# Hippogriff/prifit

Hardware: AMD Instinct MI355X
Metric: shapes/sec (fwd+bwd) B=24x2048 pts, PointNet++-MSG+ellipsoid fit (higher is better)
Workload: dtype f32; 1 GPU; configs[2]: PointNet++-MSG + mean-shift(10 it, <=25 clusters) + ellipsoid fit + convex loss, B=24x2048 per GPU, fwd+bwd+Adam; global_batch=24, points=2048, parallelism=dp1, cloud=blobs, embedding=clustered, backbone_grad_param=sa1.conv_blocks.0.0.weight, launch=eager

## Files before the change

prifit_amd/build.py:

```python
import os
import subprocess
import sys
from concurrent.futures import ThreadPoolExecutor

HERE = os.path.dirname(os.path.abspath(__file__))
ROOT = os.path.dirname(HERE)
CSRC = os.path.join(HERE, "csrc")
LIBDIR = os.path.join(HERE, "lib")
LIB = os.path.join(LIBDIR, "libprifit_hip.so")
OBJDIR = os.path.join(HERE, "build")
ARCH = "gfx950"

SOURCES = {
    "pointops.hip": ["-ffp-contract=off"],
    "sa_group.hip": ["-ffp-contract=off"],
    "gemm.hip": [],
    "gemm_stream.hip": [],
    "gemm_stream_bwd.hip": [],
    "pool_alg.hip": [],
    "sa_gather_bwd.hip": [],
    "bn.hip": [],
    "meanshift.hip": [],
    "meanshift_fused.hip": [],
    "meanshift_rows.hip": [],
    "meanshift_split.hip": [],
    "fit.hip": [],
    "fit_glue.hip": [],
    "chamfer.hip": ["-ffp-contract=off"],
    "atlas.hip": [],
    "optim.hip": [],
    "augment.hip": ["-ffp-contract=off"],
    "perturb.hip": ["-ffp-contract=off"],
    "seg_metrics.hip": [],
    "infer.hip": [],
    "infer_bf16.hip": [],
    "probe_head.hip": [],
    "edge_conv.hip": [],
    "dgcnn.hip": ["-ffp-contract=off"],
    "comm.hip": [],
}
COMMON = ["-O3", "-std=c++17", "-fPIC", "--offload-arch=" + ARCH, "-I" + os.path.join(ROOT, "include"),
          "-I" + CSRC, "-Wall", "-Wno-unused-function"] + os.environ.get("PRIFIT_BUILD_DEFS", "").split()


def _hipcc():
    for c in (os.environ.get("HIPCC"), "/opt/rocm/bin/hipcc", "hipcc"):
        if c and (os.path.isabs(c) and os.path.exists(c) or not os.path.isabs(c)):
            return c
    raise RuntimeError("hipcc not found")


def _stale(target, deps):
    if not os.path.exists(target):
        return True
    t = os.path.getmtime(target)
    return any(os.path.getmtime(d) > t for d in deps)


def build_library(force=False, verbose=False):
    import fcntl
    os.makedirs(LIBDIR, exist_ok=True)
    os.makedirs(OBJDIR, exist_ok=True)
    with open(os.path.join(LIBDIR, ".build.lock"), "w") as lock:
        fcntl.flock(lock, fcntl.LOCK_EX)
        try:
            return _build_locked(force, verbose)
        finally:
            fcntl.flock(lock, fcntl.LOCK_UN)


def _build_locked(force, verbose):
    headers = [os.path.join(CSRC, f) for f in os.listdir(CSRC) if f.endswith(".h")]
    headers.append(os.path.join(ROOT, "include", "prifit_hip.h"))
    hipcc = _hipcc()
    jobs = []
    objs = []
    for src, extra in SOURCES.items():
        s = os.path.join(CSRC, src)
        o = os.path.join(OBJDIR, src.replace(".hip", ".o"))
        objs.append(o)
        if force or _stale(o, [s] + headers):
            jobs.append([hipcc] + COMMON + extra + ["-c", s, "-o", o])

    def run(cmd):
        if verbose:
            print(" ".join(cmd), flush=True)
        r = subprocess.run(cmd, capture_output=True, text=True)
        if r.returncode != 0:
            raise RuntimeError("hipcc failed:\n%s\n%s" % (" ".join(cmd), r.stderr))
        if verbose and r.stderr.strip():
            print(r.stderr)

    if jobs:
        with ThreadPoolExecutor(max_workers=min(4, len(jobs))) as ex:
            list(ex.map(run, jobs))
    if jobs or force or _stale(LIB, objs):
        tmp = LIB + ".tmp.%d" % os.getpid()
        run([hipcc, "-shared", "-fPIC", "--offload-arch=" + ARCH, "-o", tmp] + objs + ["-ldl"])
        os.replace(tmp, LIB)
    return LIB


if __name__ == "__main__":
    print(build_library(force="--force" in sys.argv, verbose=True))
```

prifit_amd/csrc/gemm.hip:

```cpp
#include <stdlib.h>

#include <type_traits>

#include "common.h"

typedef float f32x16 __attribute__((ext_vector_type(16)));

enum { LAY_NT = 0, LAY_NN = 1, LAY_TN = 2 };
enum { EPI_NONE = 0, EPI_CHORD = 1, EPI_MSKERNEL = 2, EPI_MSBWD = 3, EPI_BNRED = 4 };

struct GemmArgs {
    const float *A, *B;
    float *C;
    int M, N, K;
    long long lda, ldb, ldc;
    long long sA, sB, sC;
    int batch, splitk;
    const float *a_scale, *a_shift;
    const float *b_scale, *b_shift;
    const float *bias;
    long long bias_stride;
    float *stats;
    int epi;
    const float *epi_batch_scalar;
    const float *aux;
    const float *row_add;
    float *a_rowsum;
    long long ldaux, sAux;
    const float *red_scale, *red_shift, *red_mean, *red_invstd;
    long long dA2, dB2;
    int kswitch;
    int accumulate;
    int vecA, vecB;
    int ntiles;
    float *cand;
};

#ifndef GEMM_W8
#define GEMM_W8 6
#endif
constexpr int BK = 32;
constexpr int PAD = 4;

__device__ __forceinline__ float4 ld4(const float *p) { return *reinterpret_cast<const float4 *>(p); }

template <int ROWS, bool KC, bool VEC, bool AFF, int NTH>
struct TileLoader {
    static constexpr int NV = ROWS * BK / 4 / NTH;
    static_assert(NV * NTH * 4 == ROWS * BK, "tile must divide evenly over the threads");
    float4 v[NV];
    const float *ptr[NV];
    int klo[NV];
    int c0[NV];
    unsigned okmask[NV];
    long long step;
    int K, R, cclamp;

    __device__ __forceinline__ void init(const float *__restrict__ base, long long ld, int r0, int R_, int K_)
    {
        K = K_; R = R_;
        step = KC ? (long long)BK : (long long)BK * ld;
#pragma unroll
        for (int p = 0; p < NV; ++p) {
            const int id = threadIdx.x + NTH * p;
            if (KC) {
                const int gr = r0 + id / (BK / 4);
                klo[p] = (id % (BK / 4)) * 4;
                okmask[p] = gr < R ? 0xFu : 0u;
                ptr[p] = base + (long long)(gr < R ? gr : 0) * ld + (klo[p] < K ? klo[p] : 0);
                c0[p] = 0;
            } else {
                klo[p] = id / (ROWS / 4);
                const int gr = r0 + (id % (ROWS / 4)) * 4;
                unsigned m = 0;
#pragma unroll
                for (int j = 0; j < 4; ++j) m |= (gr + j < R) ? (1u << j) : 0u;
                okmask[p] = m;
                c0[p] = m ? gr : 0;
                ptr[p] = base + (long long)klo[p] * ld + c0[p];
            }
        }
    }

    int kload;
    __device__ __forceinline__ void load(int k0, const float *__restrict__, const float *__restrict__)
    {
        kload = k0;
        const int kt = k0 / BK;
#pragma unroll
        for (int p = 0; p < NV; ++p) {
            const int gk = k0 + klo[p];
            const bool kin = gk < K;
            const float *src = ptr[p] + (kin ? (long long)kt * step : 0);
            if (!KC && !kin && klo[p] >= K) src = ptr[p] - (long long)klo[p] * (step / BK);
            if (VEC) {
                v[p] = ld4(src);
            } else {
                float e[4];
#pragma unroll
                for (int j = 0; j < 4; ++j) {
                    const bool ok = KC ? (okmask[p] && (gk + j) < K) : (kin && ((okmask[p] >> j) & 1u));
                    e[j] = src[ok ? j : 0];
                }
                v[p] = make_float4(e[0], e[1], e[2], e[3]);
            }
        }
    }

    __device__ __forceinline__ void finish(const float *__restrict__ scale, const float *__restrict__ shift)
    {
#pragma unroll
        for (int p = 0; p < NV; ++p) {
            const int gk = kload + klo[p];
            const bool kin = gk < K;
            float4 x = v[p];
            if (VEC) {
                if (AFF) {
                    const int cc = KC ? (kin ? gk : 0) : c0[p];
                    const float4 s = ld4(scale + cc), t = ld4(shift + cc);
                    x.x = fmaxf(fmaf(x.x, s.x, t.x), 0.f); x.y = fmaxf(fmaf(x.y, s.y, t.y), 0.f);
                    x.z = fmaxf(fmaf(x.z, s.z, t.z), 0.f); x.w = fmaxf(fmaf(x.w, s.w, t.w), 0.f);
                }
                if (!(kin && okmask[p])) x = make_float4(0.f, 0.f, 0.f, 0.f);
            } else {
                float e[4] = {x.x, x.y, x.z, x.w};
#pragma unroll
                for (int j = 0; j < 4; ++j) {
                    const bool ok = KC ? (okmask[p] && (gk + j) < K) : (kin && ((okmask[p] >> j) & 1u));
                    float val = ok ? e[j] : 0.f;
                    if (AFF && ok) {
                        const int cc = KC ? gk + j : c0[p] + j;
                        val = fmaxf(fmaf(val, scale[cc], shift[cc]), 0.f);
                    }
                    e[j] = val;
                }
                x = make_float4(e[0], e[1], e[2], e[3]);
            }
            v[p] = x;
        }
    }

    __device__ __forceinline__ void shift(long long delta)
    {
#pragma unroll
        for (int p = 0; p < NV; ++p) ptr[p] += delta;
    }

    __device__ __forceinline__ void store(float *__restrict__ lds) const
    {
#pragma unroll
        for (int p = 0; p < NV; ++p) {
            const int id = threadIdx.x + NTH * p;
            if (KC) {
                const int row = id / (BK / 4), kk = (id % (BK / 4)) * 4;
                *reinterpret_cast<float4 *>(lds + row * (BK + PAD) + kk) = v[p];
            } else {
                const int kk = id / (ROWS / 4), row = (id % (ROWS / 4)) * 4;
                *reinterpret_cast<float4 *>(lds + kk * (ROWS + PAD) + row) = v[p];
            }
        }
    }
};

typedef float f32x4v __attribute__((ext_vector_type(4)));
typedef unsigned u32x4v __attribute__((ext_vector_type(4)));
template <int ROWS, bool KC, bool AFF, int NTH>
struct ExactLoader {
    static constexpr int NV = ROWS * BK / 4 / NTH;
    static_assert(NV * NTH * 4 == ROWS * BK, "tile must divide evenly over the threads");
    float4 v[NV];
    int voff[NV];
    int klo[NV], c0[NV];
    const float *base;
    __amdgpu_buffer_rsrc_t rs;
    int step4;
    int kload;

    __device__ __forceinline__ void init(const float *__restrict__ b, long long ld, int r0, int, int)
    {
        base = b;
        rs = __builtin_amdgcn_make_buffer_rsrc(const_cast<float *>(b), 0, 0x7ffffffc, 0x00020000);
        step4 = __builtin_amdgcn_readfirstlane(KC ? BK * 4 : (int)(BK * ld * 4));
#pragma unroll
        for (int p = 0; p < NV; ++p) {
            const int id = threadIdx.x + NTH * p;
            if (KC) {
                klo[p] = (id % (BK / 4)) * 4;
                c0[p] = 0;
                voff[p] = (int)(((long long)(r0 + id / (BK / 4)) * ld + klo[p]) * 4);
            } else {
                klo[p] = id / (ROWS / 4);
                c0[p] = r0 + (id % (ROWS / 4)) * 4;
                voff[p] = (int)(((long long)klo[p] * ld + c0[p]) * 4);
            }
        }
    }
    __device__ __forceinline__ void load(int k0, const float *__restrict__, const float *__restrict__)
    {
        kload = k0;
        const int soff = __builtin_amdgcn_readfirstlane((k0 / BK) * step4);
#pragma unroll
        for (int p = 0; p < NV; ++p) {
            const f32x4v t = __builtin_bit_cast(f32x4v, __builtin_amdgcn_raw_buffer_load_b128(rs, voff[p], soff, 0));
            v[p] = make_float4(t.x, t.y, t.z, t.w);
        }
    }
    __device__ __forceinline__ void finish(const float *__restrict__ scale, const float *__restrict__ shift)
    {
        if (!AFF) return;
#pragma unroll
        for (int p = 0; p < NV; ++p) {
            const int cc = KC ? kload + klo[p] : c0[p];
            const float4 s = ld4(scale + cc), t = ld4(shift + cc);
            float4 x = v[p];
            x.x = fmaxf(fmaf(x.x, s.x, t.x), 0.f); x.y = fmaxf(fmaf(x.y, s.y, t.y), 0.f);
            x.z = fmaxf(fmaf(x.z, s.z, t.z), 0.f); x.w = fmaxf(fmaf(x.w, s.w, t.w), 0.f);
            v[p] = x;
        }
    }
    __device__ __forceinline__ void shift(long long delta)
    {
        base += delta;
        rs = __builtin_amdgcn_make_buffer_rsrc(const_cast<float *>(base), 0, 0x7ffffffc, 0x00020000);
    }
    __device__ __forceinline__ void store(float *__restrict__ lds) const
    {
#pragma unroll
        for (int p = 0; p < NV; ++p) {
            const int id = threadIdx.x + NTH * p;
            if (KC) {
                const int row = id / (BK / 4), kk = (id % (BK / 4)) * 4;
                *reinterpret_cast<float4 *>(lds + row * (BK + PAD) + kk) = v[p];
            } else {
                const int kk = id / (ROWS / 4), row = (id % (ROWS / 4)) * 4;
                *reinterpret_cast<float4 *>(lds + kk * (ROWS + PAD) + row) = v[p];
            }
        }
    }
};

template <int ROWS, bool KC, bool AFF, int NTH>
struct BufLoader {
    static constexpr int NV = ROWS * BK / 4 / NTH;
    static_assert(NV * NTH * 4 == ROWS * BK, "tile must divide evenly over the threads");
    static constexpr int OOBV = 0x7fffffff;
    float4 v[NV];
    int voff[NV];
    int klo[NV], c0[NV];
    __amdgpu_buffer_rsrc_t rs;
    const float *base;
    int step4, K, kload;

    __device__ __forceinline__ void init(const float *__restrict__ b, long long ld, int r0, int R, int K_)
    {
        K = K_;
        base = b;
        rs = __builtin_amdgcn_make_buffer_rsrc(const_cast<float *>(b), 0, 0x7ffffffc, 0x00020000);
        step4 = KC ? BK * 4 : (int)(BK * ld * 4);
#pragma unroll
        for (int p = 0; p < NV; ++p) {
            const int id = threadIdx.x + NTH * p;
            if (KC) {
                const int row = r0 + id / (BK / 4);
                klo[p] = (id % (BK / 4)) * 4;
                c0[p] = 0;
                voff[p] = row < R ? (int)(((long long)row * ld + klo[p]) * 4) : OOBV;
            } else {
                klo[p] = id / (ROWS / 4);
                c0[p] = r0 + (id % (ROWS / 4)) * 4;
                voff[p] = c0[p] < R ? (int)(((long long)klo[p] * ld + c0[p]) * 4) : OOBV;
                if (c0[p] >= R) c0[p] = 0;
            }
        }
    }
    __device__ __forceinline__ void load(int k0, const float *__restrict__, const float *__restrict__) { load(k0); }
    __device__ __forceinline__ void shift(long long delta)
    {
        base += delta;
        rs = __builtin_amdgcn_make_buffer_rsrc(const_cast<float *>(base), 0, 0x7ffffffc, 0x00020000);
    }
    __device__ __forceinline__ void load(int k0)
    {
        kload = k0;
        const int soff = (k0 / BK) * step4;
        if (k0 + BK <= K) {
#pragma unroll
            for (int p = 0; p < NV; ++p) {
                const f32x4v t = __builtin_bit_cast(f32x4v, __builtin_amdgcn_raw_buffer_load_b128(rs, voff[p], soff, 0));
                v[p] = make_float4(t.x, t.y, t.z, t.w);
            }
        } else {
#pragma unroll
            for (int p = 0; p < NV; ++p) {
                const int vo = k0 + klo[p] < K ? voff[p] : OOBV;
                const f32x4v t = __builtin_bit_cast(f32x4v, __builtin_amdgcn_raw_buffer_load_b128(rs, vo, soff, 0));
                v[p] = make_float4(t.x, t.y, t.z, t.w);
            }
        }
    }
    __device__ __forceinline__ void finish(const float *__restrict__ scale, const float *__restrict__ shift)
    {
        if (!AFF) return;
#pragma unroll
        for (int p = 0; p < NV; ++p) {
            const int gk = kload + klo[p];
            const bool ok = voff[p] != OOBV && gk < K;
            const int cc = KC ? (gk < K ? gk : 0) : c0[p];
// ... 420 lines not shown
            const float bias = (g.bias && cok) ? g.bias[col] : 0.f;
            float rs = 0.f, rt = 0.f, rmu = 0.f, ris = 0.f;
            if (RED && cok) { rs = g.red_scale[col]; rt = g.red_shift[col]; rmu = g.red_mean[col]; ris = g.red_invstd[col]; }
            const int c_voff = cok ? (int)(((long long)rbase * g.ldc + col) * 4) : 0x7fffffff;
            const int y_voff = (RED && cok) ? (int)(((long long)rbase * g.ldaux + col) * 4) : 0x7fffffff;
            float kf[16];
            if (RED) {
#pragma unroll
                for (int r = 0; r < 16; ++r) {
                    const int ro = ((r & 3) + 8 * (r >> 2)) * ldy4;
                    kf[r] = __builtin_bit_cast(float, full_rows ? __builtin_amdgcn_raw_buffer_load_b32(yrs, y_voff, ro, 0)
                                                                 : __builtin_amdgcn_raw_buffer_load_b32(yrs, cok ? y_voff + ro : y_voff, 0, 0));
                }
            }
            float vmax = -INFINITY, vmin = INFINITY, v0 = 0.f;
            int imax = 0, imin = 0;
#pragma unroll
            for (int r = 0; r < 16; ++r) {
                const int row = rbase + (r & 3) + 8 * (r >> 2);
                const float v = acc[b][r] + bias;
                const float vs = (cok && (full_rows || row < g.M)) ? v : 0.f;
                if (PMAX) {
                    const int ri = (r & 3) + 8 * (r >> 2) + 4 * lh;
                    const bool rok = full_rows || row < g.M;
                    if (rok && v > vmax) { vmax = v; imax = ri; }
                    if (rok && v < vmin) { vmin = v; imin = ri; }
                }
                if (RED) {
                    const float gm = fmaf(kf[r], rs, rt) > 0.f ? vs : 0.f;
                    csum[b] += gm;
                    csq[b] += gm * ((kf[r] - rmu) * ris);
                } else {
                    csum[b] += vs;
                    if (r == 0) v0 = vs;
                    else if (r == 1) csq[b] = fmaf(v0, v0, vs * vs);
                    else csq[b] = fmaf(vs, vs, csq[b]);
                }
                {
                    const int ro = ((r & 3) + 8 * (r >> 2)) * ldc4;
                    if (full_rows) __builtin_amdgcn_raw_buffer_store_b32(__builtin_bit_cast(unsigned, v), crs, c_voff, ro, 0);
                    else __builtin_amdgcn_raw_buffer_store_b32(__builtin_bit_cast(unsigned, v), crs, cok ? c_voff + ro : c_voff, 0, 0);
                }
            }
            if (PMAX) {
                const float ov = __shfl_xor(vmax, 32, 64), on = __shfl_xor(vmin, 32, 64);
                const int oi = __shfl_xor(imax, 32, 64), oj = __shfl_xor(imin, 32, 64);
                if (ov > vmax || (ov == vmax && oi < imax)) { vmax = ov; imax = oi; }
                if (on < vmin || (on == vmin && oj < imin)) { vmin = on; imin = oj; }
                const int blk_row = m0 + wm0;
                if (lh == 0 && cok && blk_row < g.M) {
                    float *cd = g.cand + (long long)(blk_row >> 5) * 4 * g.N + col;
                    cd[0] = vmax; cd[g.N] = __int_as_float(imax); cd[2 * g.N] = vmin; cd[3 * g.N] = __int_as_float(imin);
                }
            }
        }
        PERS_STAMP(3);
        if (g.stats) {
            float *red = lds;
#pragma unroll
            for (int b = 0; b < TN; ++b) {
                const float s = csum[b] + __shfl_xor(csum[b], 32, 64);
                const float q = csq[b] + __shfl_xor(csq[b], 32, 64);
                if (lh == 0) {
                    red[(wmi * 2 + 0) * BN + wn0 + 32 * b + li] = s;
                    red[(wmi * 2 + 1) * BN + wn0 + 32 * b + li] = q;
                }
            }
            __syncthreads();
            for (int t = threadIdx.x; t < 2 * BN; t += NTH) {
                const int which = t / BN, c = t - which * BN;
                float s = 0.f;
#pragma unroll
                for (int w = 0; w < BM / WM; ++w) s += red[(w * 2 + which) * BN + c];
                if (n0 + c < g.N) g.stats[((long long)tile_m * 2 + which) * g.N + n0 + c] = s;
            }
            if (has_next) __syncthreads();
        }
        PERS_STAMP(4);
        if (!has_next) break;
        tix = ntix; tile_m = ntile_m; tile_n = ntile_n;
        la.finish(g.a_scale, g.a_shift);
        la.store(lds); lb.store(lds + SZA);
        __syncthreads();
        PERS_STAMP(5);
#ifdef PERS_STAMPS
        ++st_tile;
#endif
    }
}

#ifndef CHORD_XCD
#define CHORD_XCD 1
#endif
template <int MODE>
__global__ __launch_bounds__(512) __attribute__((amdgpu_waves_per_eu(4, 4))) void chord_sym_kernel(
    const float *__restrict__ A, long long lda, long long sA, float *__restrict__ C, long long ldc, long long sC, int n, int K,
    int batch, unsigned long long *__restrict__ okey, const float *__restrict__ thr, unsigned *__restrict__ mask)
{
    constexpr bool GRAM = MODE == 1, MASK = MODE == 2;
    constexpr int BM = 128, BN = 128, WM = 32, WN = 64, NTH = 512, TN = WN / 32, WAVES_N = BN / WN;
    constexpr int SZ = BM * (BK + PAD);
    constexpr int TLD = BM + 4;
    __shared__ __attribute__((aligned(16))) float lds[4 * SZ];
    static_assert(4 * SZ >= BN * TLD, "the transposed tile fits the staging buffers");
    const int T = n / BM;
    int t, zb;
#if CHORD_XCD
    xcd_shape_block((int)blockIdx.x, T * (T + 1) / 2, batch, zb, t);
#else
    t = (int)blockIdx.x % (T * (T + 1) / 2); zb = (int)blockIdx.x / (T * (T + 1) / 2);
#endif
    int tile_m = 0;
    while (t >= T - tile_m) { t -= T - tile_m; ++tile_m; }
    const int tile_n = tile_m + t;
    const int m0 = tile_m * BM, n0 = tile_n * BN;
    const float *Az = A + (long long)zb * sA;
    float *Cz = MASK ? nullptr : C + (long long)zb * sC;
    const int MW = n / 32;
    unsigned *Mz = MASK ? mask + (long long)zb * n * MW : nullptr;
    const float th = MASK ? thr[zb] : 0.f;
    const int wave = __builtin_amdgcn_readfirstlane(threadIdx.x >> 6), lane = threadIdx.x & 63;
    const int li = lane & 31, lh = lane >> 5;
    const int wm0 = (wave / WAVES_N) * WM, wn0 = (wave % WAVES_N) * WN;

    BufLoader<BM, true, false, NTH> la, lb;
    la.init(Az, lda, m0, n, K);
    lb.init(Az, lda, n0, n, K);
    const int ktiles = K / BK;
    la.load(0); lb.load(0);
    la.store(lds); lb.store(lds + SZ);
    __syncthreads();
    f32x16 acc[TN];
#pragma unroll
    for (int b = 0; b < TN; ++b)
#pragma unroll
        for (int r = 0; r < 16; ++r) acc[b][r] = 0.f;
    for (int kt = 0; kt < ktiles; ++kt) {
        const int stage = kt & 1;
        const float *As = lds + stage * 2 * SZ, *Bs = As + SZ;
        const bool more = kt + 1 < ktiles;
        if (more) { la.load((kt + 1) * BK); lb.load((kt + 1) * BK); }
#pragma unroll
        for (int gk = 0; gk < BK / 8; ++gk) {
            const float4 fa = read_frag<BM, true>(As, wm0 + li, gk, lh);
            float4 fb[TN];
#pragma unroll
            for (int b = 0; b < TN; ++b) fb[b] = read_frag<BN, true>(Bs, wn0 + 32 * b + li, gk, lh);
#pragma unroll
            for (int b = 0; b < TN; ++b) {
                acc[b] = __builtin_amdgcn_mfma_f32_32x32x2f32(fa.x, fb[b].x, acc[b], 0, 0, 0);
                acc[b] = __builtin_amdgcn_mfma_f32_32x32x2f32(fa.y, fb[b].y, acc[b], 0, 0, 0);
                acc[b] = __builtin_amdgcn_mfma_f32_32x32x2f32(fa.z, fb[b].z, acc[b], 0, 0, 0);
                acc[b] = __builtin_amdgcn_mfma_f32_32x32x2f32(fa.w, fb[b].w, acc[b], 0, 0, 0);
            }
        }
        if (more) {
            float *An = lds + (stage ^ 1) * 2 * SZ;
            la.store(An); lb.store(An + SZ);
        }
        __syncthreads();
    }
    const bool mirror = tile_m != tile_n;
    unsigned long long *okz = okey ? okey + (long long)zb * n : nullptr;
    auto fkey = [](float f) { const unsigned u = __float_as_uint(f); return (u & 0x80000000u) ? ~u : (u | 0x80000000u); };
#pragma unroll
    for (int b = 0; b < TN; ++b) {
        const int col = wn0 + 32 * b + li;
        float cmin = INFINITY;
        int cidx = 0;
#pragma unroll
        for (int r = 0; r < 16; ++r) {
            const int row = wm0 + (r & 3) + 8 * (r >> 2) + 4 * lh;
            const float v = GRAM ? acc[b][r] : 2.0f - 2.0f * acc[b][r];
            if (MASK) {
                const unsigned long long m = __ballot(v < th);
                if (li == 0) Mz[(long long)(m0 + row) * MW + (n0 + wn0 + 32 * b) / 32] = lh ? (unsigned)(m >> 32) : (unsigned)m;
            } else {
                Cz[(long long)(m0 + row) * ldc + n0 + col] = v;
            }
            if (mirror) lds[col * TLD + row] = v;
            if (v < cmin) { cmin = v; cidx = row; }
        }
        if (okz) {
            const float ov = __shfl_xor(cmin, 32, 64);
            const int oi = __shfl_xor(cidx, 32, 64);
            if (ov < cmin || (ov == cmin && oi < cidx)) { cmin = ov; cidx = oi; }
            if (lh == 0) atomicMin(okz + n0 + col, ((unsigned long long)fkey(cmin) << 32) | (unsigned)(m0 + cidx));
        }
    }
    if (mirror) {
        __syncthreads();
        if (MASK) {
            static_assert(BN * (BM / 32) == NTH, "one word per thread");
            const int trow = threadIdx.x / (BM / 32), w = threadIdx.x - trow * (BM / 32);
            unsigned bits = 0;
#pragma unroll
            for (int q = 0; q < 8; ++q) {
                const float4 v = *reinterpret_cast<const float4 *>(lds + trow * TLD + 32 * w + 4 * q);
                bits |= (unsigned)(v.x < th) << (4 * q) | (unsigned)(v.y < th) << (4 * q + 1) | (unsigned)(v.z < th) << (4 * q + 2) |
                        (unsigned)(v.w < th) << (4 * q + 3);
            }
            Mz[(long long)(n0 + trow) * MW + m0 / 32 + w] = bits;
        } else
        for (int i = threadIdx.x; i < BN * (BM / 4); i += NTH) {
            const int trow = i / (BM / 4), c4 = i - trow * (BM / 4);
            *reinterpret_cast<float4 *>(Cz + (long long)(n0 + trow) * ldc + m0 + 4 * c4) =
                *reinterpret_cast<const float4 *>(lds + trow * TLD + 4 * c4);
        }
        if (okz) {
            const int r = threadIdx.x & (BM - 1), q = threadIdx.x >> 7;
            float rmin = INFINITY;
            int ridx = 0;
#pragma unroll 8
            for (int c = 32 * q; c < 32 * q + 32; ++c) {
                const float v = lds[c * TLD + r];
                if (v < rmin) { rmin = v; ridx = c; }
            }
            atomicMin(okz + m0 + r, ((unsigned long long)fkey(rmin) << 32) | (unsigned)(n0 + ridx));
        }
    }
}

template <bool FB>
__global__ __launch_bounds__(512) __attribute__((amdgpu_waves_per_eu(4, 4))) void gemm_tnsk_kernel(const GemmArgs g)
{
    constexpr int BM = 128, BN = 128, WM = 32, WN = 64, NTH = 512, TN = WN / 32;
    constexpr int SZA = BK * (BM + PAD), SZB = BK * (BN + PAD);
    __shared__ __attribute__((aligned(16))) float lds[2 * (SZA + SZB)];
    const int tilesN = (g.N + BN - 1) / BN;
    const int tile_m = blockIdx.x / tilesN, tile_n = blockIdx.x - tile_m * tilesN;
    const int m0 = tile_m * BM, n0 = tile_n * BN;
    const int ktiles = (g.K + BK - 1) / BK;
    const int per = (ktiles + g.splitk - 1) / g.splitk;
    const int kt0 = blockIdx.z * per, kt1 = min(ktiles, kt0 + per);
    if (kt0 >= kt1) return;
    const int wave = __builtin_amdgcn_readfirstlane(threadIdx.x >> 6), lane = threadIdx.x & 63;
    const int li = lane & 31, lh = lane >> 5;
    const int wm0 = (wave % (BM / WM)) * WM, wn0 = (wave / (BM / WM)) * WN;
    const int nbv = m0 + wm0 >= g.M ? 0 : min(TN, max(0, (g.N - n0 - wn0 + 31) >> 5));

    BufLoader<BM, false, false, NTH> la[2];
    BufLoader<BN, false, FB, NTH> lb[2];
#pragma unroll
    for (int i = 0; i < 2; ++i) { la[i].init(g.A, g.lda, m0, g.M, g.K); lb[i].init(g.B, g.ldb, n0, g.N, g.K); }
    la[0].load(kt0 * BK); lb[0].load(kt0 * BK);
    if (kt0 + 1 < kt1) { la[1].load((kt0 + 1) * BK); lb[1].load((kt0 + 1) * BK); }
    lb[0].finish(g.b_scale, g.b_shift);
    la[0].store(lds); lb[0].store(lds + SZA);
    __syncthreads();
    f32x16 acc[TN];
#pragma unroll
    for (int b = 0; b < TN; ++b)
#pragma unroll
        for (int r = 0; r < 16; ++r) acc[b][r] = 0.f;
    auto step = [&](int kt, auto par) {
        constexpr int S = decltype(par)::value;
        const float *As = lds + S * (SZA + SZB), *Bs = As + SZA;
        if (kt + 2 < kt1) { la[S].load((kt + 2) * BK); lb[S].load((kt + 2) * BK); }
        __builtin_amdgcn_sched_barrier(0);
        mma_ktile<BM, false, BN, false, TN>(As, Bs, wm0 + li, wn0 + li, lh, acc, BK / 8, nbv);
        if (kt + 1 < kt1) {
            float *An = lds + (S ^ 1) * (SZA + SZB);
            lb[S ^ 1].finish(g.b_scale, g.b_shift);
            la[S ^ 1].store(An); lb[S ^ 1].store(An + SZA);
        }
        __syncthreads();
    };
    int kt = kt0;
    for (; kt + 1 < kt1; kt += 2) {
        step(kt, std::integral_constant<int, 0>());
        step(kt + 1, std::integral_constant<int, 1>());
    }
    if (kt < kt1) step(kt, std::integral_constant<int, 0>());
    const int rbase = m0 + wm0 + 4 * lh;
#pragma unroll
    for (int b = 0; b < TN; ++b) {
        const int col = n0 + wn0 + 32 * b + li;
        if (col >= g.N) continue;
#pragma unroll
        for (int r = 0; r < 16; ++r) {
            const int row = rbase + (r & 3) + 8 * (r >> 2);
            if (row >= g.M) continue;
            float *dst = g.C + (long long)row * g.ldc + col;
            if (g.splitk > 1) unsafeAtomicAdd(dst, acc[b][r]);
            else if (g.accumulate) *dst += acc[b][r];
            else *dst = acc[b][r];
        }
    }
}

static bool launch_tnsk(const GemmArgs &g, hipStream_t st)
{
    if (g.batch != 1 || g.a_scale || g.bias || g.stats || g.epi != EPI_NONE || g.a_rowsum || g.kswitch ||
        !(g.vecA && g.vecB) || (g.M & 3) || (g.N & 3) || (g.splitk > 1 && !g.accumulate) || g.splitk > 65535)
        return false;
    const long long lim = 0x7ff00000LL;
    if ((long long)g.K * g.lda * 4 >= lim || (long long)g.K * g.ldb * 4 >= lim) return false;
    const dim3 grid(((g.M + 127) / 128) * ((g.N + 127) / 128), 1, g.splitk), block(512);
    if (g.b_scale) hipLaunchKernelGGL((gemm_tnsk_kernel<true>), grid, block, 0, st, g);
    else hipLaunchKernelGGL((gemm_tnsk_kernel<false>), grid, block, 0, st, g);
    return true;
}

static bool launch_persistent(const GemmArgs &g_, int lay, hipStream_t st, float *want_cand = nullptr, bool dry = false)
{
    GemmArgs g = g_;
    if (lay == LAY_TN || g.batch != 1 || g.splitk != 1 || g.accumulate || g.a_rowsum || g.kswitch ||
        g.b_scale || !(g.epi == EPI_NONE || g.epi == EPI_BNRED) || !(g.vecA && g.vecB) || (g.K & 3) || (lay == LAY_NN && (g.N & 3)))
        return false;
    const long long lim = 0x7ff00000LL;
    if ((long long)g.M * g.lda * 4 >= lim || (long long)(lay == LAY_NT ? g.N : g.K) * g.ldb * 4 >= lim ||
        (long long)g.M * g.ldc * 4 >= lim || (g.epi == EPI_BNRED && (long long)g.M * g.ldaux * 4 >= lim))
        return false;
    g.ntiles = ((g.M + 127) / 128) * ((g.N + 127) / 128);
    const int slots = 512;
    if (g.ntiles <= slots) return false;
    if (dry) return lay == LAY_NT && g.epi == EPI_NONE && g.a_scale;
    const dim3 grid(slots), block(512);
    if (lay == LAY_NT) {
        if (g.epi != EPI_NONE) return false;
        if (want_cand) {
            g.cand = want_cand;
            if (g.a_scale) hipLaunchKernelGGL((gemm_pers_kernel<LAY_NT, true, false, true>), grid, block, 0, st, g);
            else hipLaunchKernelGGL((gemm_pers_kernel<LAY_NT, false, false, true>), grid, block, 0, st, g);
        } else if (g.a_scale) hipLaunchKernelGGL((gemm_pers_kernel<LAY_NT, true, false>), grid, block, 0, st, g);
        else hipLaunchKernelGGL((gemm_pers_kernel<LAY_NT, false, false>), grid, block, 0, st, g);
    } else {
        if (want_cand) return false;
        if (g.a_scale) return false;
        if (g.epi == EPI_BNRED) hipLaunchKernelGGL((gemm_pers_kernel<LAY_NN, false, true>), grid, block, 0, st, g);
        else hipLaunchKernelGGL((gemm_pers_kernel<LAY_NN, false, false>), grid, block, 0, st, g);
    }
    return true;
}

__global__ __launch_bounds__(512, 4) void gemm_dual_sk_kernel(const GemmArgs g)
{
    constexpr int BM = 128, BN = 128, WN = 64, NTH = 512, TN = 2, WAVES_N = 2;
    constexpr int SZA = BM * (BK + PAD), SZB = BK * (BN + PAD);
    __shared__ __attribute__((aligned(16))) float lds[2 * (SZA + SZB)];
    const int tilesM = g.M / BM;
    const int ktiles = g.K / BK;
    const long long total = (long long)g.batch * tilesM * ktiles;
    int u = (int)(total * blockIdx.x / gridDim.x);
    const int uend = (int)(total * (blockIdx.x + 1) / gridDim.x);
    const int wave = threadIdx.x >> 6, lane = threadIdx.x & 63;
    const int li = lane & 31, lh = lane >> 5;
    const int wm0 = (wave / WAVES_N) * 32, wn0 = (wave % WAVES_N) * WN;
    const int kswitch = g.kswitch ? g.kswitch : 0x7fffffff;

    while (u < uend) {
        const int t = u / ktiles;
        const int kt0 = u - t * ktiles, kt1 = min(ktiles, kt0 + (uend - u));
        const int z = t / tilesM, tile_m = t - z * tilesM;
        const int m0 = tile_m * BM;
        const float *A = g.A + (long long)z * g.sA;
        const float *B = g.B + (long long)z * g.sB;
        float *C = g.C + (long long)z * g.sC;

        f32x16 acc[TN];
#pragma unroll
        for (int b = 0; b < TN; ++b)
#pragma unroll
            for (int r = 0; r < 16; ++r) acc[b][r] = 0.f;
        ExactLoader<BM, true, false, NTH> la;
        ExactLoader<BN, false, false, NTH> lb;
        la.init(A, g.lda, m0, g.M, g.K);
        lb.init(B, g.ldb, 0, g.N, g.K);
        if (kt0 >= kswitch) { la.shift(g.dA2); lb.shift(g.dB2); }
        la.load(kt0 * BK, nullptr, nullptr);
        lb.load(kt0 * BK, nullptr, nullptr);
        la.store(lds);
        lb.store(lds + SZA);
        __syncthreads();
        for (int kt = kt0; kt < kt1; ++kt) {
            const int stage = (kt - kt0) & 1;
            const float *As = lds + stage * (SZA + SZB), *Bs = As + SZA;
            const bool more = kt + 1 < kt1;
            if (more) {
                if (kt + 1 == kswitch) { la.shift(g.dA2); lb.shift(g.dB2); }
                la.load((kt + 1) * BK, nullptr, nullptr);
                lb.load((kt + 1) * BK, nullptr, nullptr);
            }
            mma_ktile<BM, true, BN, false, TN>(As, Bs, wm0 + li, wn0 + li, lh, acc);
            if (more) {
                float *An = lds + (stage ^ 1) * (SZA + SZB);
                la.store(An);
                lb.store(An + SZA);
            }
            __syncthreads();
        }
        const int rbase = m0 + wm0 + 4 * lh;
#pragma unroll
        for (int b = 0; b < TN; ++b) {
            const int col = wn0 + 32 * b + li;
#pragma unroll
            for (int r = 0; r < 16; ++r)
                unsafeAtomicAdd(C + (long long)(rbase + (r & 3) + 8 * (r >> 2)) * g.ldc + col, acc[b][r]);
        }
        u += kt1 - kt0;
    }
}

template <int BM, int BN, int WM, int WN, int LAY, bool VEC>
static void launch_aff(const GemmArgs &g, dim3 grid, hipStream_t st)
{
    const dim3 block((BM / WM) * (BN / WN) * 64);
    const long long spanA = (LAY == LAY_TN ? (long long)g.K * g.lda : (long long)g.M * g.lda) * 4;
    const long long spanB = (LAY == LAY_NT ? (long long)g.N * g.ldb : (long long)g.K * g.ldb) * 4;
    const bool exact = VEC && !g.a_rowsum && spanA < 0x7ff00000LL && spanB < 0x7ff00000LL;
    if (exact) {
        if (g.a_scale) hipLaunchKernelGGL((gemm_kernel<BM, BN, WM, WN, LAY, true, true, true, false, true>), grid, block, 0, st, g);
        else if (g.b_scale) hipLaunchKernelGGL((gemm_kernel<BM, BN, WM, WN, LAY, true, true, false, true, true>), grid, block, 0, st, g);
        else hipLaunchKernelGGL((gemm_kernel<BM, BN, WM, WN, LAY, true, true, false, false, true>), grid, block, 0, st, g);
        return;
    }
    if (g.a_scale) hipLaunchKernelGGL((gemm_kernel<BM, BN, WM, WN, LAY, VEC, VEC, true, false>), grid, block, 0, st, g);
    else if (g.b_scale) hipLaunchKernelGGL((gemm_kernel<BM, BN, WM, WN, LAY, VEC, VEC, false, true>), grid, block, 0, st, g);
    else hipLaunchKernelGGL((gemm_kernel<BM, BN, WM, WN, LAY, VEC, VEC, false, false>), grid, block, 0, st, g);
}

template <int BM, int BN, int WM, int WN>
static int launch_cfg(const GemmArgs &g, int lay, hipStream_t st)
{
    const int tilesM = (g.M + BM - 1) / BM, tilesN = (g.N + BN - 1) / BN;
    dim3 grid(tilesM * tilesN, 1, g.batch * g.splitk);
    const bool vec = g.vecA && g.vecB;
    if (g.a_scale && g.b_scale) return PRIFIT_EINVAL;
    switch (lay) {
        case LAY_NT:
            if (vec) launch_aff<BM, BN, WM, WN, LAY_NT, true>(g, grid, st);
            else launch_aff<BM, BN, WM, WN, LAY_NT, false>(g, grid, st);
            break;
        case LAY_NN:
            if (vec) launch_aff<BM, BN, WM, WN, LAY_NN, true>(g, grid, st);
            else launch_aff<BM, BN, WM, WN, LAY_NN, false>(g, grid, st);
            break;
        default:
            if (vec) launch_aff<BM, BN, WM, WN, LAY_TN, true>(g, grid, st);
            else launch_aff<BM, BN, WM, WN, LAY_TN, false>(g, grid, st);
            break;
    }
    return prifit_check_launch();
}

static inline bool aligned16(const void *p) { return ((uintptr_t)p & 15) == 0; }

static inline bool small_tiles(int M, int N, int batch, int splitk)
{
    const long long wgs = (long long)((M + 127) / 128) * ((N + 127) / 128) * batch * splitk;
    return wgs < (splitk > 1 ? 160 : 520) && M > 64 && N > 32;
}

static int dispatch(GemmArgs &g, int layout, void *stream)
{
    const int M = g.M, N = g.N, K = g.K;
    const int extA = layout == LAY_TN ? M : K, extB = layout == LAY_NT ? K : N;
    g.vecA = aligned16(g.A) && (g.lda % 4 == 0) && (g.sA % 4 == 0) && (extA % 4 == 0);
    g.vecB = aligned16(g.B) && (g.ldb % 4 == 0) && (g.sB % 4 == 0) && (extB % 4 == 0);
    hipStream_t st = as_stream(stream);
    if (small_tiles(M, N, g.batch, g.splitk)) return launch_cfg<64, 64, 32, 32>(g, layout, st);
    if (N <= 32) return launch_cfg<128, 32, 32, 32>(g, layout, st);
    if (N <= 64) return launch_cfg<128, 64, 32, 64>(g, layout, st);
    if (N <= 96) return launch_cfg<128, 96, 32, 96>(g, layout, st);
    if (launch_persistent(g, layout, st)) return prifit_check_launch();
    if (layout == LAY_TN && launch_tnsk(g, st)) return prifit_check_launch();
    return launch_cfg<128, 128, 32, 64>(g, layout, st);
}

extern "C" {

#ifdef PERS_STAMPS
int prifit_debug_pers_ktail(int on)
{
    return hipMemcpyToSymbol(HIP_SYMBOL(g_pers_ktail), &on, sizeof(int)) == hipSuccess ? 0 : -1;
}
int prifit_debug_pers_stamps(unsigned long long *host, int n)
{
    return hipMemcpyFromSymbol(host, HIP_SYMBOL(g_pers_stamps), sizeof(unsigned long long) * (size_t)n) == hipSuccess ? 0 : -1;
}
#endif

int prifit_gemm_tile_m(int N)
{
    (void)N;
    return 128;
}

int prifit_gemm_stats_tile_m(int M, int N)
{
    return small_tiles(M, N, 1, 1) ? 64 : 128;
}

int prifit_gemm_f32(int layout, int M, int N, int K, const float *A, long long lda, long long strideA,
                    const float *B, long long ldb, long long strideB, float *C, long long ldc,
                    long long strideC, int batch, int splitk, const float *a_scale, const float *a_shift,
                    const float *b_scale, const float *b_shift, const float *bias, long long bias_batch_stride,
                    float *col_stats, int epilogue, const float *epi_batch_scalar, const float *epi_aux, long long ld_aux,
                    long long stride_aux, const float *epi_row_add, float *a_rowsum, int accumulate, void *stream)
{
    if (!A || !B || !C || M <= 0 || N <= 0 || K <= 0 || batch <= 0 || splitk <= 0 || layout < 0 || layout > 2 ||
        (epilogue != 100 && (epilogue < 0 || epilogue > 3)) || (epilogue >= EPI_MSKERNEL && !epi_batch_scalar) ||
        (epilogue == EPI_MSBWD && !epi_aux) || (splitk > 1 && !accumulate) ||
        ((a_scale == nullptr) != (a_shift == nullptr)) || ((b_scale == nullptr) != (b_shift == nullptr)) ||
        (col_stats && (batch != 1 || splitk != 1)) || (epilogue != EPI_NONE && epilogue != 100 && splitk != 1) || (long long)batch * splitk > 65535)
        return PRIFIT_EINVAL;
    GemmArgs g;
    g.A = A; g.B = B; g.C = C; g.M = M; g.N = N; g.K = K;
    g.lda = lda; g.ldb = ldb; g.ldc = ldc; g.sA = strideA; g.sB = strideB; g.sC = strideC;
    g.batch = batch; g.splitk = splitk;
    g.a_scale = a_scale; g.a_shift = a_shift; g.b_scale = b_scale; g.b_shift = b_shift;
    g.bias = bias; g.bias_stride = bias_batch_stride; g.stats = col_stats; g.epi = epilogue; g.epi_batch_scalar = epi_batch_scalar;
    g.accumulate = accumulate; g.aux = epi_aux; g.ldaux = ld_aux; g.sAux = stride_aux;
    g.row_add = epi_row_add; g.a_rowsum = a_rowsum;
    g.red_scale = g.red_shift = g.red_mean = g.red_invstd = nullptr;
    g.dA2 = g.dB2 = 0; g.kswitch = 0;
    if (a_rowsum && (layout == LAY_TN || splitk != 1)) return PRIFIT_EINVAL;
    return dispatch(g, layout, stream);
}

int prifit_gemm_dual_nn_f32(int M, int N, int K1, int K2, const float *A1, const float *A2, long long lda,
                            long long strideA, const float *B1, const float *B2, long long ldb, long long strideB,
                            float *C, long long ldc, long long strideC, int batch, int splitk, int accumulate,
                            void *stream)
{
    if (!A1 || !A2 || !B1 || !B2 || !C || M <= 0 || N <= 0 || K1 <= 0 || K2 <= 0 || (K1 % BK) || batch <= 0 ||
        splitk <= 0 || (splitk > 1 && !accumulate) || (long long)batch * splitk > 65535 || lda < K1 || lda < K2 ||
        ldb < N || ldc < N)
        return PRIFIT_EINVAL;
    if ((((uintptr_t)A1 ^ (uintptr_t)A2) | ((uintptr_t)B1 ^ (uintptr_t)B2)) & 15) return PRIFIT_EINVAL;
    GemmArgs g;
    g.A = A1; g.B = B1; g.C = C; g.M = M; g.N = N; g.K = K1 + K2;
    g.lda = lda; g.ldb = ldb; g.ldc = ldc; g.sA = strideA; g.sB = strideB; g.sC = strideC;
    g.batch = batch; g.splitk = splitk;
    g.a_scale = g.a_shift = g.b_scale = g.b_shift = nullptr;
    g.bias = nullptr; g.bias_stride = 0; g.stats = nullptr; g.epi = EPI_NONE; g.epi_batch_scalar = nullptr;
    g.accumulate = accumulate; g.aux = nullptr; g.ldaux = 0; g.sAux = 0; g.row_add = nullptr; g.a_rowsum = nullptr;
    g.red_scale = g.red_shift = g.red_mean = g.red_invstd = nullptr;
    g.dA2 = (A2 - A1) - (long long)K1;
    g.dB2 = (B2 - B1) - (long long)K1 * ldb;
    g.kswitch = K1 / BK;
    if (accumulate && N == 128 && M % 128 == 0 && K1 == K2 && aligned16(A1) && aligned16(B1) && (lda % 4 == 0) &&
        (ldb % 4 == 0) && (strideA % 4 == 0) && (strideB % 4 == 0) && (long long)M * lda * 4 < 0x7ff00000LL &&
        (long long)(K1 + K2) * ldb * 4 < 0x7ff00000LL) {
        static const int slots = [] {
            int dev = 0;
            hipDeviceProp_t p;
            if (hipGetDevice(&dev) != hipSuccess || hipGetDeviceProperties(&p, dev) != hipSuccess) return 512;
            return 2 * p.multiProcessorCount;
        }();
        const long long total = (long long)batch * (M / 128) * ((K1 + K2) / BK);
        const int grid = (int)(total < slots ? total : slots);
        hipLaunchKernelGGL(gemm_dual_sk_kernel, dim3(grid), dim3(512), 0, as_stream(stream), g);
        return prifit_check_launch();
    }
    return dispatch(g, LAY_NN, stream);
}

int prifit_gemm_dgrad_bnred_f32(int M, int N, int K, const float *dY, long long lda, const float *W, long long ldb,
                                float *G, long long ldc, const float *Yprev, long long ldy, const float *scale,
                                const float *shift, const float *mean, const float *invstd, float *red_slab, void *stream)
{
    if (!dY || !W || !G || !Yprev || !scale || !shift || !mean || !invstd || !red_slab || M <= 0 || N <= 0 || K <= 0 ||
        lda < K || ldb < N || ldc < N || ldy < N)
        return PRIFIT_EINVAL;
    GemmArgs g;
    g.A = dY; g.B = W; g.C = G; g.M = M; g.N = N; g.K = K;
    g.lda = lda; g.ldb = ldb; g.ldc = ldc; g.sA = g.sB = g.sC = 0;
    g.batch = 1; g.splitk = 1;
    g.a_scale = g.a_shift = g.b_scale = g.b_shift = nullptr;
    g.bias = nullptr; g.bias_stride = 0; g.stats = red_slab; g.epi = EPI_BNRED; g.epi_batch_scalar = nullptr;
    g.accumulate = 0; g.aux = Yprev; g.ldaux = ldy; g.sAux = 0; g.row_add = nullptr; g.a_rowsum = nullptr;
    g.red_scale = scale; g.red_shift = shift; g.red_mean = mean; g.red_invstd = invstd;
    g.dA2 = g.dB2 = 0; g.kswitch = 0;
    return dispatch(g, LAY_NN, stream);
}

int prifit_chord_sym_f32(const float *A, long long lda, long long strideA, float *C, long long ldc, long long strideC,
                         int n, int K, int batch, unsigned long long *owner_key, void *stream)
{
    if (!A || !C || n <= 0 || (n % 128) || K <= 0 || (K % BK) || batch <= 0 || batch > 65535 || lda < K || ldc < n || (lda & 3) ||
        (ldc & 3) || (strideA & 3) || (strideC & 3) || ((uintptr_t)A & 15) || ((uintptr_t)C & 15) ||
        (long long)n * lda * 4 >= 0x7ff00000LL)
        return PRIFIT_EINVAL;
    const int T = n / 128;
    hipLaunchKernelGGL(chord_sym_kernel<0>, dim3((unsigned)(T * (T + 1) / 2 * batch)), dim3(512), 0, as_stream(stream), A, lda,
                       strideA, C, ldc, strideC, n, K, batch, owner_key, (const float *)nullptr, (unsigned *)nullptr);
    return prifit_check_launch();
}

int prifit_chord_sym_mask(const float *A, long long lda, long long strideA, const float *thr, uint32_t *mask, int n, int K, int batch,
                          unsigned long long *owner_key, void *stream)
{
    if (!A || !thr || !mask || n <= 0 || (n % 128) || K <= 0 || (K % BK) || batch <= 0 || batch > 65535 || lda < K || (lda & 3) ||
        (strideA & 3) || ((uintptr_t)A & 15) || (long long)n * lda * 4 >= 0x7ff00000LL)
        return PRIFIT_EINVAL;
    const int T = n / 128;
    hipLaunchKernelGGL(chord_sym_kernel<2>, dim3((unsigned)(T * (T + 1) / 2 * batch)), dim3(512), 0, as_stream(stream), A, lda,
                       strideA, (float *)nullptr, 0LL, 0LL, n, K, batch, owner_key, thr, mask);
    return prifit_check_launch();
}

int prifit_gram_sym_f32(const float *A, long long lda, long long strideA, float *C, long long ldc, long long strideC, int n, int K,
                        int batch, void *stream)
{
    if (!A || !C || n <= 0 || (n % 128) || K <= 0 || (K % BK) || batch <= 0 || batch > 65535 || lda < K || ldc < n || (lda & 3) ||
        (ldc & 3) || (strideA & 3) || (strideC & 3) || ((uintptr_t)A & 15) || ((uintptr_t)C & 15) ||
        (long long)n * lda * 4 >= 0x7ff00000LL)
        return PRIFIT_EINVAL;
    const int T = n / 128;
    hipLaunchKernelGGL(chord_sym_kernel<1>, dim3((unsigned)(T * (T + 1) / 2 * batch)), dim3(512), 0, as_stream(stream), A, lda,
                       strideA, C, ldc, strideC, n, K, batch, (unsigned long long *)nullptr, (const float *)nullptr, (unsigned *)nullptr);
    return prifit_check_launch();
}

static void pool_gemm_args(GemmArgs &g, int M, int N, int K, const float *A, long long lda, const float *W, long long ldb,
                           float *Y, long long ldc, const float *a_scale, const float *a_shift, const float *bias, float *stats)
{
    g.A = A; g.B = W; g.C = Y; g.M = M; g.N = N; g.K = K; g.lda = lda; g.ldb = ldb; g.ldc = ldc;
    g.sA = g.sB = g.sC = 0; g.batch = 1; g.splitk = 1;
// ... 33 lines not shown
```

Baseline: 1642 shapes/s.

## Add persistent row-block MFMA GEMM kernel for narrow-N NT layers

Adds a persistent GEMM kernel that gives each workgroup 128 full rows across the whole output width (N up to 256, K up to 256). It double-buffers the weight slice in LDS and prefetches the next A tile in registers, and fuses the input affine+ReLU, bias, BN statistics and the max/min candidate epilogue. It is dispatched from the persistent NT path for specific N/K ranges. The aim is to cut repeated B loads and tile-scheduling overhead for the narrow pointwise-conv GEMMs in the MLPs. The cost is high register pressure from holding up to 8 accumulators of 16 floats each, with waves_per_eu forced to 2.

```diff
diff --git a/prifit_amd/build.py b/prifit_amd/build.py
--- a/prifit_amd/build.py
+++ b/prifit_amd/build.py
@@ -15,6 +15,7 @@
     "pointops.hip": ["-ffp-contract=off"],
     "sa_group.hip": ["-ffp-contract=off"],
     "gemm.hip": [],
+    "gemm_rowblock.hip": [],
     "gemm_stream.hip": [],
     "gemm_stream_bwd.hip": [],
     "pool_alg.hip": [],
diff --git a/prifit_amd/csrc/gemm.hip b/prifit_amd/csrc/gemm.hip
--- a/prifit_amd/csrc/gemm.hip
+++ b/prifit_amd/csrc/gemm.hip
@@ -3,6 +3,7 @@
 #include <type_traits>
 
 #include "common.h"
+#include "gemm_rowblock.h"
 
 typedef float f32x16 __attribute__((ext_vector_type(16)));
 
@@ -1029,6 +1030,19 @@
     return true;
 }
 
+static bool launch_rowblock(const GemmArgs &g, int lay, hipStream_t st, float *want_cand)
+{
+    static const bool on = [] {
+        const char *e = getenv("PRIFIT_GEMM_ROWBLOCK");
+        return !(e && e[0] == '0');
+    }();
+    if (!on || lay != LAY_NT || g.epi != EPI_NONE) return false;
+    RowBlockArgs r;
+    r.A = g.A; r.B = g.B; r.C = g.C; r.M = g.M; r.N = g.N; r.K = g.K; r.lda = g.lda; r.ldb = g.ldb; r.ldc = g.ldc;
+    r.a_scale = g.a_scale; r.a_shift = g.a_shift; r.bias = g.bias; r.stats = g.stats; r.cand = want_cand;
+    return prifit_rowblock_launch(r, st);
+}
+
 static bool launch_persistent(const GemmArgs &g_, int lay, hipStream_t st, float *want_cand = nullptr, bool dry = false)
 {
     GemmArgs g = g_;
@@ -1043,6 +1057,7 @@
     const int slots = 512;
     if (g.ntiles <= slots) return false;
     if (dry) return lay == LAY_NT && g.epi == EPI_NONE && g.a_scale;
+    if (launch_rowblock(g, lay, st, want_cand)) return true;
     const dim3 grid(slots), block(512);
     if (lay == LAY_NT) {
         if (g.epi != EPI_NONE) return false;
diff --git a/prifit_amd/csrc/gemm_rowblock.h b/prifit_amd/csrc/gemm_rowblock.h
--- /dev/null
+++ b/prifit_amd/csrc/gemm_rowblock.h
@@ -0,0 +1,15 @@
+#pragma once
+#include <hip/hip_runtime.h>
+
+struct RowBlockArgs {
+    const float *A, *B;
+    float *C;
+    int M, N, K;
+    long long lda, ldb, ldc;
+    const float *a_scale, *a_shift;
+    const float *bias;
+    float *stats;
+    float *cand;
+};
+
+bool prifit_rowblock_launch(const RowBlockArgs &g, hipStream_t st);
diff --git a/prifit_amd/csrc/gemm_rowblock.hip b/prifit_amd/csrc/gemm_rowblock.hip
--- /dev/null
+++ b/prifit_amd/csrc/gemm_rowblock.hip
@@ -0,0 +1,272 @@
+#include "common.h"
+#include "gemm_rowblock.h"
+
+typedef float f32x16 __attribute__((ext_vector_type(16)));
+typedef float f32x4v __attribute__((ext_vector_type(4)));
+
+namespace {
+
+constexpr int RB_BK = 32;
+constexpr int RB_NTH = 256;
+constexpr int RB_KMAX = 256;
+constexpr int RB_OOB = 0x7fffffff;
+
+__device__ __forceinline__ __amdgpu_buffer_rsrc_t rb_rsrc(const float *p, long long bytes)
+{
+    return __builtin_amdgcn_make_buffer_rsrc(const_cast<float *>(p), 0, (int)bytes, 0x00020000);
+}
+
+template <int NB>
+struct WSlice {
+    static constexpr int ROWS = 32 * NB;
+    static constexpr int LD = RB_BK + 4;
+    static constexpr int SZ = ROWS * LD;
+    static constexpr int NV = NB;
+    static constexpr int NH = (NV + 1) / 2;
+    f32x4v v[NH];
+    int voff, kof, n0, N, K;
+    int stepp4;
+
+    __device__ __forceinline__ void init(long long ldb, int N_, int K_)
+    {
+        K = K_; N = N_;
+        n0 = threadIdx.x / (RB_BK / 4);
+        kof = (threadIdx.x % (RB_BK / 4)) * 4;
+        voff = (int)(((long long)n0 * ldb + kof) * 4);
+        stepp4 = (int)(32 * ldb * 4);
+    }
+    template <int P0, int P1>
+    __device__ __forceinline__ void load(__amdgpu_buffer_rsrc_t rs, int kt)
+    {
+        const bool kin = kt * RB_BK + kof < K;
+#pragma unroll
+        for (int p = P0; p < P1; ++p) {
+            const int vo = (n0 + 32 * p < N && kin) ? voff + p * stepp4 + kt * RB_BK * 4 : RB_OOB;
+            v[p - P0] = __builtin_bit_cast(f32x4v, __builtin_amdgcn_raw_buffer_load_b128(rs, vo, 0, 0));
+        }
+    }
+    template <int P0, int P1>
+    __device__ __forceinline__ void store(float *__restrict__ lds) const
+    {
+#pragma unroll
+        for (int p = P0; p < P1; ++p)
+            *reinterpret_cast<f32x4v *>(lds + (threadIdx.x / (RB_BK / 4) + 32 * p) * LD + (threadIdx.x % (RB_BK / 4)) * 4) = v[p - P0];
+    }
+    static __device__ __forceinline__ f32x4v frag(const float *__restrict__ lds, int b, int g, int li, int lh)
+    {
+        return *reinterpret_cast<const f32x4v *>(lds + (32 * b + li) * LD + 8 * g + 4 * lh);
+    }
+};
+
+template <int NB, bool PMAX>
+__global__ __launch_bounds__(RB_NTH) __attribute__((amdgpu_waves_per_eu(2, 2))) void gemm_rowblock_kernel(const RowBlockArgs g)
+{
+    typedef WSlice<NB> WS;
+    constexpr int SZB = WS::SZ, ROWS = WS::ROWS;
+    __shared__ __attribute__((aligned(16))) float s_w[2 * SZB];
+    __shared__ __attribute__((aligned(16))) float s_aff[2 * RB_KMAX];
+    static_assert(4 * 2 * ROWS <= SZB, "the statistics of the four waves fit one stage");
+
+    const int wave = __builtin_amdgcn_readfirstlane(threadIdx.x >> 6), lane = threadIdx.x & 63;
+    const int li = lane & 31, lh = lane >> 5;
+    const int ktiles = (g.K + RB_BK - 1) / RB_BK;
+    const int ngk_last = (g.K - (ktiles - 1) * RB_BK + 7) >> 3;
+    const int nblocks = (g.M + 127) >> 7;
+    const bool fa = g.a_scale != nullptr;
+
+    for (int t = threadIdx.x; t < 2 * RB_KMAX; t += RB_NTH) {
+        const int k = t & (RB_KMAX - 1);
+        s_aff[t] = (fa && k < g.K) ? (t < RB_KMAX ? g.a_scale[k] : g.a_shift[k]) : 0.f;
+    }
+
+    const __amdgpu_buffer_rsrc_t ars = rb_rsrc(g.A, ((long long)(g.M - 1) * g.lda + g.K) * 4);
+    const __amdgpu_buffer_rsrc_t wrs = rb_rsrc(g.B, ((long long)(g.N - 1) * g.ldb + g.K) * 4);
+    const __amdgpu_buffer_rsrc_t crs = rb_rsrc(g.C, g.C ? ((long long)(g.M - 1) * g.ldc + g.N) * 4 : 0);
+    const int ldc4 = (int)g.ldc * 4;
+
+    auto a_voff = [&](int rb) {
+        const int row = rb * 128 + wave * 32 + li;
+        return row < g.M ? (int)(((long long)row * g.lda + 4 * lh) * 4) : RB_OOB;
+    };
+    f32x4v an[4];
+    auto a_load = [&](int voff, int kt) {
+        if ((kt + 1) * RB_BK <= g.K) {
+            const int soff = __builtin_amdgcn_readfirstlane(kt * RB_BK * 4);
+#pragma unroll
+            for (int gk = 0; gk < 4; ++gk)
+                an[gk] = __builtin_bit_cast(f32x4v, __builtin_amdgcn_raw_buffer_load_b128(ars, voff, soff + gk * 32, 0));
+        } else {
+#pragma unroll
+            for (int gk = 0; gk < 4; ++gk) {
+                const int k0 = kt * RB_BK + 8 * gk;
+                const int vo = (voff != RB_OOB && k0 + 4 * lh < g.K) ? voff + k0 * 4 : RB_OOB;
+                an[gk] = __builtin_bit_cast(f32x4v, __builtin_amdgcn_raw_buffer_load_b128(ars, vo, 0, 0));
+            }
+        }
+    };
+
+    WS lw;
+    lw.init(g.ldb, g.N, g.K);
+    int rb = blockIdx.x;
+    constexpr int NH = WS::NH, NV = WS::NV;
+    lw.template load<0, NH>(wrs, 0);
+    a_load(a_voff(rb), 0);
+    lw.template store<0, NH>(s_w);
+    lw.template load<NH, NV>(wrs, 0);
+    lw.template store<NH, NV>(s_w);
+    __syncthreads();
+
+    int it = 0;
+    for (;;) {
+        const int nrb = rb + (int)gridDim.x;
+        const bool has_next = nrb < nblocks;
+        f32x16 acc[NB];
+#pragma unroll
+        for (int b = 0; b < NB; ++b)
+#pragma unroll
+            for (int r = 0; r < 16; ++r) acc[b][r] = 0.f;
+        const int voff_cur = a_voff(rb);
+        for (int kt = 0; kt < ktiles; ++kt, ++it) {
+            const float *Ws = s_w + (it & 1) * SZB;
+            f32x4v ac[4];
+#pragma unroll
+            for (int gk = 0; gk < 4; ++gk) {
+                ac[gk] = an[gk];
+                if (fa) {
+                    const f32x4v s = *reinterpret_cast<const f32x4v *>(s_aff + kt * RB_BK + 8 * gk + 4 * lh);
+                    const f32x4v h = *reinterpret_cast<const f32x4v *>(s_aff + RB_KMAX + kt * RB_BK + 8 * gk + 4 * lh);
+#pragma unroll
+                    for (int j = 0; j < 4; ++j) ac[gk][j] = fmaxf(fmaf(ac[gk][j], s[j], h[j]), 0.f);
+                }
+            }
+            const bool more = kt + 1 < ktiles;
+            const bool fill = more || has_next;
+            const int nkt = more ? kt + 1 : 0;
+            float *Wn = s_w + ((it + 1) & 1) * SZB;
+            if (fill) {
+                a_load(more ? voff_cur : a_voff(nrb), nkt);
+                lw.template load<0, NH>(wrs, nkt);
+            }
+            __builtin_amdgcn_sched_barrier(0);
+            const int ngk = more ? RB_BK / 8 : ngk_last;
+            f32x4v fb[2];
+            fb[0] = WS::frag(Ws, 0, 0, li, lh);
+#pragma unroll
+            for (int gk = 0; gk < RB_BK / 8; ++gk) {
+                if (gk > 0 && gk >= ngk) break;
+#pragma unroll
+                for (int b = 0; b < NB; ++b) {
+                    const int s = gk * NB + b;
+                    if (s + 1 < NB * (RB_BK / 8)) fb[(s + 1) & 1] = WS::frag(Ws, (b + 1) % NB, gk + (b + 1) / NB, li, lh);
+                    __builtin_amdgcn_sched_barrier(0);
+                    const f32x4v a = ac[gk], w = fb[s & 1];
+                    acc[b] = __builtin_amdgcn_mfma_f32_32x32x2f32(a.x, w.x, acc[b], 0, 0, 0);
+                    acc[b] = __builtin_amdgcn_mfma_f32_32x32x2f32(a.y, w.y, acc[b], 0, 0, 0);
+                    acc[b] = __builtin_amdgcn_mfma_f32_32x32x2f32(a.z, w.z, acc[b], 0, 0, 0);
+                    acc[b] = __builtin_amdgcn_mfma_f32_32x32x2f32(a.w, w.w, acc[b], 0, 0, 0);
+                    __builtin_amdgcn_sched_barrier(0);
+                }
+                if (gk == 0 && fill) {
+                    lw.template store<0, NH>(Wn);
+                    lw.template load<NH, NV>(wrs, nkt);
+                    __builtin_amdgcn_sched_barrier(0);
+                }
+            }
+            if (fill) lw.template store<NH, NV>(Wn);
+            __syncthreads();
+        }
+
+        const int row0 = rb * 128 + wave * 32;
+        const bool full_rows = row0 + 32 <= g.M;
+        const int rbase = row0 + 4 * lh;
+        float *red = s_w + ((it + 1) & 1) * SZB;
+#pragma unroll
+        for (int b = 0; b < NB; ++b) {
+            const int col = 32 * b + li;
+            const bool cok = col < g.N;
+            int colv = col;
+            asm volatile("" : "+v"(colv));
+            const float bias = (g.bias && cok) ? g.bias[colv] : 0.f;
+            const int c_voff = cok ? (int)(((long long)rbase * g.ldc + col) * 4) : RB_OOB;
+            float csum = 0.f, csq = 0.f;
+            float vmax = -INFINITY, vmin = INFINITY;
+            int imax = 0, imin = 0;
+#pragma unroll
+            for (int r = 0; r < 16; ++r) {
+                const int rr = (r & 3) + 8 * (r >> 2);
+                const bool rok = full_rows || rbase + rr < g.M;
+                const float v = acc[b][r] + bias;
+                const float vs = (cok && rok) ? v : 0.f;
+                if (PMAX) {
+                    const int ri = rr + 4 * lh;
+                    if (rok && v > vmax) { vmax = v; imax = ri; }
+                    if (rok && v < vmin) { vmin = v; imin = ri; }
+                }
+                csum += vs;
+                csq = fmaf(vs, vs, csq);
+                if (full_rows) __builtin_amdgcn_raw_buffer_store_b32(__builtin_bit_cast(unsigned, v), crs, c_voff, rr * ldc4, 0);
+                else __builtin_amdgcn_raw_buffer_store_b32(__builtin_bit_cast(unsigned, v), crs, (cok && rok) ? c_voff + rr * ldc4 : RB_OOB, 0, 0);
+            }
+            if (PMAX) {
+                const float ov = __shfl_xor(vmax, 32, 64), on = __shfl_xor(vmin, 32, 64);
+                const int oi = __shfl_xor(imax, 32, 64), oj = __shfl_xor(imin, 32, 64);
+                if (ov > vmax || (ov == vmax && oi < imax)) { vmax = ov; imax = oi; }
+                if (on < vmin || (on == vmin && oj < imin)) { vmin = on; imin = oj; }
+                if (lh == 0 && cok && row0 < g.M) {
+                    float *cd = g.cand + (long long)(row0 >> 5) * 4 * g.N + col;
+                    cd[0] = vmax; cd[g.N] = __int_as_float(imax); cd[2 * g.N] = vmin; cd[3 * g.N] = __int_as_float(imin);
+                }
+            }
+            if (g.stats) {
+                const float s = csum + __shfl_xor(csum, 32, 64);
+                const float q = csq + __shfl_xor(csq, 32, 64);
+                if (lh == 0) { red[(wave * 2 + 0) * ROWS + col] = s; red[(wave * 2 + 1) * ROWS + col] = q; }
+            }
+        }
+        if (g.stats) {
+            __syncthreads();
+            for (int t = threadIdx.x; t < 2 * ROWS; t += RB_NTH) {
+                const int which = t / ROWS, c = t - which * ROWS;
+                float s = 0.f;
+#pragma unroll
+                for (int w = 0; w < 4; ++w) s += red[(w * 2 + which) * ROWS + c];
+                if (c < g.N) g.stats[((long long)rb * 2 + which) * g.N + c] = s;
+            }
+            __syncthreads();
+        }
+        if (!has_next) break;
+        rb = nrb;
+    }
+}
+
+template <int NB>
+void launch_nb(const RowBlockArgs &g, dim3 grid, hipStream_t st)
+{
+    if (g.cand) hipLaunchKernelGGL((gemm_rowblock_kernel<NB, true>), grid, dim3(RB_NTH), 0, st, g);
+    else hipLaunchKernelGGL((gemm_rowblock_kernel<NB, false>), grid, dim3(RB_NTH), 0, st, g);
+}
+
+int resident_slots()
+{
+    static const int n = [] {
+        int dev = 0;
+        hipDeviceProp_t p;
+        if (hipGetDevice(&dev) != hipSuccess || hipGetDeviceProperties(&p, dev) != hipSuccess) return 512;
+        return 2 * p.multiProcessorCount;
+    }();
+    return n;
+}
+
+}
+
+bool prifit_rowblock_launch(const RowBlockArgs &g, hipStream_t st)
+{
+    const int NB = (g.N + 31) / 32;
+    const bool take = (NB == 7 && g.K > 96 && g.K <= 128) || (NB == 8 && g.K > 128 && g.K <= RB_KMAX);
+    if (!take || g.M < 128) return false;
+    const int nblocks = (g.M + 127) / 128, slots = resident_slots();
+    const dim3 grid(nblocks < slots ? nblocks : slots);
+    if (NB == 7) launch_nb<7>(g, grid, st);
+    else launch_nb<8>(g, grid, st);
+    return true;
+}
```

Result: no change. 1649 shapes/s (median of 6 runs) (+0.4%).
